# likojack/bnv_fusion

Measured on AMD Instinct MI355X. Metric: depth frames/sec fused+decoded, 640x480 @ 256^3 grid, higher is better.
Workload: dtype f32 operands split into f16 hi+lo, 3 products on v_mfma_f32_16x16x32_f16, f32 accumulate

## Files before the change

### bnv_fusion_amd/csrc/encode_mlp.hip

```cpp
#include "encode.hpp"

namespace bnv {

__device__ __forceinline__ f32x16 relu16(f32x16 v) {
#pragma unroll
  for (int r = 0; r < 16; ++r) v[r] = relu_bits(v[r]);
  return v;
}

__device__ __forceinline__ f32x16 bias_init(const float* __restrict__ b, int mb, int h) {
  f32x16 v;
#pragma unroll
  for (int q = 0; q < 4; ++q) {
    const f32x4 t = *(const f32x4*)&b[mb * 32 + 8 * q + 4 * h];
#pragma unroll
    for (int i = 0; i < 4; ++i) v[4 * q + i] = t[i];
  }
  return v;
}

__device__ __forceinline__ void layer128(const float* __restrict__ wp, const float* __restrict__ bias,
                                         const f32x16 (&in)[4], f32x16 (&out)[4], int lane, int h) {
#pragma unroll
  for (int mb = 0; mb < 4; ++mb) out[mb] = bias_init(bias, mb, h);
#pragma unroll
  for (int nb = 0; nb < 4; ++nb) {
#pragma unroll
    for (int rq = 0; rq < 4; ++rq) {
      f32x4 a[4];
#pragma unroll
      for (int mb = 0; mb < 4; ++mb)
        a[mb] = *(const f32x4*)&wp[(((mb * 4 + nb) * 4 + rq) * 64 + lane) * 4];
#pragma unroll
      for (int i = 0; i < 4; ++i) {
#pragma unroll
        for (int mb = 0; mb < 4; ++mb)
          out[mb] = __builtin_amdgcn_mfma_f32_32x32x2f32(a[mb][i], in[nb][4 * rq + i], out[mb], 0, 0, 0);
      }
    }
  }
}

__global__ __launch_bounds__(512, 2) void k_pointnet_scatter(
    const float* __restrict__ pts, int n_points, bnv_grid_t g, const float* __restrict__ wpack,
    const uint32_t* __restrict__ bitmap, const uint32_t* __restrict__ word_prefix,
    int32_t* __restrict__ counts, long long* __restrict__ acc, const int32_t* __restrict__ pair_list,
    const int32_t* __restrict__ n_pairs) {
  extern __shared__ __attribute__((aligned(16))) float lds[];
  stage_to_lds<512>(wpack, lds, PN_TOTAL * 4);
  __syncthreads();

  const int lane = threadIdx.x & 63;
  const int wave = __builtin_amdgcn_readfirstlane(threadIdx.x >> 6);
  const int j = lane & 31, h = lane >> 5;
  const PairTiles T = pair_tiles(n_points, pair_list, n_pairs);
  const int n_tiles = T.n_tiles;

  for (int t = blockIdx.x * 8 + wave; t < n_tiles; t += gridDim.x * 8) {
    int i = 0, k = 0;
    const bool have = tile_pair(T, t, j, &i, &k);
    float in0 = 0.f, in1 = 0.f, in2 = 0.f;
    int slot = -1;
    bool valid = false;
    if (have) {
      const float* p = pts + (size_t)i * 6;
      const float x = p[0], y = p[1], z = p[2];
      valid = in_bounds(x, y, z, g);
      if (valid) {
        const float xn = voxel_coord(x, g.bound_min[0], g.voxel_size);
        const float yn = voxel_coord(y, g.bound_min[1], g.voxel_size);
        const float zn = voxel_coord(z, g.bound_min[2], g.voxel_size);
        int gx, gy, gz;
        const uint32_t id = corner_voxel(k, xn, yn, zn, g, gx, gy, gz);
        if (voxel_owner(gx, gy, gz, g) == g.shard_rank) slot = slot_rank(bitmap[id >> 5], word_prefix[id >> 5], id);
        const float rx = relative_coord(xn, gx, g.voxel_size);
        const float ry = relative_coord(yn, gy, g.voxel_size);
        const float rz = relative_coord(zn, gz, g.voxel_size);
        in0 = h ? ry : rx;
        in1 = h ? p[3] : rz;
        in2 = h ? p[5] : p[4];
      }
    }
    if (__ballot(slot >= 0) == 0ULL) continue;

    f32x16 ha[4], hb[4];
#pragma unroll
    for (int mb = 0; mb < 4; ++mb) ha[mb] = bias_init(lds + PN_B1, mb, h);
    {
      const float bin[3] = {in0, in1, in2};
#pragma unroll
      for (int s = 0; s < 3; ++s) {
#pragma unroll
        for (int mb = 0; mb < 4; ++mb)
          ha[mb] = __builtin_amdgcn_mfma_f32_32x32x2f32(lds[PN_W1 + (s * 4 + mb) * 64 + lane], bin[s],
                                                        ha[mb], 0, 0, 0);
      }
    }
#pragma unroll
    for (int mb = 0; mb < 4; ++mb) ha[mb] = relu16(ha[mb]);
    layer128(lds + PN_W2, lds + PN_B2, ha, hb, lane, h);
#pragma unroll
    for (int mb = 0; mb < 4; ++mb) hb[mb] = relu16(hb[mb]);
    layer128(lds + PN_W3, lds + PN_B3, hb, ha, lane, h);
#pragma unroll
    for (int mb = 0; mb < 4; ++mb) ha[mb] = relu16(ha[mb]);
    f32x16 o;
#pragma unroll
    for (int r = 0; r < 16; ++r) o[r] = 0.f;
    {
      const f32x4 b4 = *(const f32x4*)&lds[PN_B4 + 4 * h];
#pragma unroll
      for (int r = 0; r < 4; ++r) o[r] = b4[r];
    }
#pragma unroll
    for (int nb = 0; nb < 4; ++nb) {
#pragma unroll
      for (int rq = 0; rq < 4; ++rq) {
        f32x4 a = {0.f, 0.f, 0.f, 0.f};
        if (j < 8) a = *(const f32x4*)&lds[PN_W4 + ((((nb * 4 + rq) * 2 + h) * 8) + j) * 4];
#pragma unroll
        for (int i = 0; i < 4; ++i)
          o = __builtin_amdgcn_mfma_f32_32x32x2f32(a[i], ha[nb][4 * rq + i], o, 0, 0, 0);
      }
    }
    scatter_tile(o, slot, j, h, counts, acc);
  }
}

typedef __attribute__((address_space(3))) const half8 lds_half8_t;
typedef __attribute__((address_space(3))) const f32x4 lds_f32x4_t;
constexpr int kLdsWin = 61440;

#ifdef BNV_PHASE_PROF
__device__ unsigned long long g_enc_phase[8 * 16];
#define BNV_EPH(i)                                                                          \
  do {                                                                                      \
    if ((threadIdx.x & 63) == 0) {                                                          \
      unsigned long long* _p = (unsigned long long*)((char*)lds + PX_LDS_BYTES) + (threadIdx.x >> 6) * 16; \
      const unsigned long long _t = clock64();                                              \
      _p[i] += _t - _p[15];                                                                 \
      _p[15] = _t;                                                                          \
    }                                                                                       \
  } while (0)
constexpr int kEncProfLds = 8 * 16 * 8;
#else
#define BNV_EPH(i)
constexpr int kEncProfLds = 0;
#endif

struct EncLdsX {
  uint32_t w[3];
  uint32_t b;
};
__device__ __forceinline__ half8 ldsx_wfrag(const EncLdsX& L, int byte_off) {
  const int b = byte_off / kLdsWin;
  return *(lds_half8_t*)((b == 0 ? L.w[0] : (b == 1 ? L.w[1] : L.w[2])) + (uint32_t)(byte_off - b * kLdsWin));
}
__device__ __forceinline__ f32x4 ldsx_bias(const EncLdsX& L, int layer, int rb) {
  return *(lds_f32x4_t*)(L.b + (uint32_t)((layer * 128 + rb * 16) * 4));
}

template <int NPROD>
__device__ __forceinline__ void layer128_x(const EncLdsX& L, int w_off, int layer, const half8 (&inh)[4][2],
                                           const half8 (&inl)[4][2], f32x4 (&out)[8][2]) {
#pragma unroll
  for (int rb = 0; rb < 8; ++rb) out[rb][0] = out[rb][1] = ldsx_bias(L, layer, rb);
  half8 ah[2], al[2];
#define BNV_LOAD_WX(q)                                                        \
  {                                                                           \
    const int wb = (w_off + (q) * 2 * 64 * 8) * 2;                            \
    ah[(q) & 1] = ldsx_wfrag(L, wb);                                          \
    if (NPROD == 3) al[(q) & 1] = ldsx_wfrag(L, wb + 1024);                   \
  }
  BNV_LOAD_WX(0);
#pragma unroll
  for (int q = 0; q < 32; ++q) {
    if (q + 1 < 32) BNV_LOAD_WX(q + 1);
    __builtin_amdgcn_sched_barrier(0);
    const int s = q >> 3, rb = q & 7;
    if constexpr (NPROD == 3) {
      out[rb][0] = __builtin_amdgcn_mfma_f32_16x16x32_f16(al[q & 1], inh[s][0], out[rb][0], 0, 0, 0);
      out[rb][1] = __builtin_amdgcn_mfma_f32_16x16x32_f16(al[q & 1], inh[s][1], out[rb][1], 0, 0, 0);
      out[rb][0] = __builtin_amdgcn_mfma_f32_16x16x32_f16(ah[q & 1], inl[s][0], out[rb][0], 0, 0, 0);
      out[rb][1] = __builtin_amdgcn_mfma_f32_16x16x32_f16(ah[q & 1], inl[s][1], out[rb][1], 0, 0, 0);
    }
    out[rb][0] = __builtin_amdgcn_mfma_f32_16x16x32_f16(ah[q & 1], inh[s][0], out[rb][0], 0, 0, 0);
    out[rb][1] = __builtin_amdgcn_mfma_f32_16x16x32_f16(ah[q & 1], inh[s][1], out[rb][1], 0, 0, 0);
    __builtin_amdgcn_sched_barrier(0);
  }
#undef BNV_LOAD_WX
}

template <int NPROD>
__device__ __forceinline__ void split_x(const f32x4 (&acc)[8][2], half8 (&oh)[4][2], half8 (&ol)[4][2]) {
#pragma unroll
  for (int s = 0; s < 4; ++s)
#pragma unroll
    for (int cb = 0; cb < 2; ++cb) {
      float x[8];
#pragma unroll
      for (int e = 0; e < 8; ++e) x[e] = relu_bits(acc[2 * s + (e >> 2)][cb][e & 3]);
      if (NPROD == 3) {
        split8_f16(x, oh[s][cb], ol[s][cb]);
      } else {
#pragma unroll
        for (int e = 0; e < 8; ++e) oh[s][cb][e] = (_Float16)x[e];
      }
    }
}

__device__ __forceinline__ void scatter_tile_x(const f32x4& o, int slot, int n, int g, int32_t* __restrict__ counts,
                                               long long* __restrict__ acc) {
  uint32_t lo[4], hi[4];
#pragma unroll
  for (int q = 0; q < 4; ++q) fixed_hi_lo(o[q], hi[q], lo[q]);
  asm volatile(BNV_SCAN_ROWS : BNV_SCAN_REGS(lo, hi) : : "vcc");
  {
    const int tsrc = ((g & 1) * 16 + 15) * 4;
#pragma unroll
    for (int q = 0; q < 4; ++q) {
      const uint32_t tl = (uint32_t)__builtin_amdgcn_ds_bpermute(tsrc, (int)lo[q]);
      const uint32_t th = (uint32_t)__builtin_amdgcn_ds_bpermute(tsrc, (int)hi[q]);
      if (g >= 2) {
        const unsigned long long v = (((unsigned long long)hi[q] << 32) | lo[q]) + (((unsigned long long)th << 32) | tl);
        lo[q] = (uint32_t)v;
        hi[q] = (uint32_t)(v >> 32);
      }
    }
  }
  const int p = (g >> 1) * 16 + n;
  const int slot15 = __builtin_amdgcn_readlane(slot, 15);
  const int prev_row = __builtin_amdgcn_update_dpp(0, slot, 0x111 , 0xf, 0xf, false);
  const int prev = n == 0 ? slot15 : prev_row;
  const unsigned long long heads64 = __ballot(p == 0 || prev != slot);
  const uint32_t heads = ((uint32_t)heads64 & 0xffffu) | (((uint32_t)(heads64 >> 32) & 0xffffu) << 16);
  const int s = 31 - __clz((int)(heads & (0xffffffffu >> (31 - p))));
  const bool is_end = p == 31 || ((heads >> (p + 1)) & 1u);
  const int sp = s > 0 ? s - 1 : 0;
  const int src = (((sp >> 4) * 2 + (g & 1)) * 16 + (sp & 15)) * 4;
  uint32_t plo[4], phi[4];
#pragma unroll
  for (int q = 0; q < 4; ++q) {
    plo[q] = (uint32_t)__builtin_amdgcn_ds_bpermute(src, (int)lo[q]);
    phi[q] = (uint32_t)__builtin_amdgcn_ds_bpermute(src, (int)hi[q]);
  }
#ifdef BNV_PROBE_NO_SCATTER
  if ((blockIdx.x & 63) != 0) return;
#endif
  if (slot >= 0 && is_end) {
    unsigned long long* dst = (unsigned long long*)acc + ((uint32_t)slot * 8u + 4u * (uint32_t)(g & 1));
#pragma unroll
    for (int q = 0; q < 4; ++q) {
      unsigned long long v = ((unsigned long long)hi[q] << 32) | lo[q];
      if (s > 0) v -= ((unsigned long long)phi[q] << 32) | plo[q];
      atomicAdd(dst + q, v);
    }
    if ((g & 1) == 0) atomicAdd(&counts[slot], p - s + 1);
  }
}

template <int NPROD>
__global__ __launch_bounds__(512, 2) __attribute__((amdgpu_num_vgpr(120))) void k_pointnet_scatter_x(
    const float* __restrict__ pts, int n_points, bnv_grid_t g, const float* __restrict__ wpack,
    const uint32_t* __restrict__ bitmap, const uint32_t* __restrict__ word_prefix,
    int32_t* __restrict__ counts, long long* __restrict__ acc, int32_t* __restrict__ error,
    const int32_t* __restrict__ pair_list, const int32_t* __restrict__ n_pairs) {
  extern __shared__ __attribute__((aligned(16))) float lds[];
  const float n_cert = wpack[PN_CERT];
  float* lb = lds + PX_TOTAL / 2;
  for (int i = threadIdx.x; i < 128 * 3 + 8; i += 512) lb[i] = wpack[PN_B1 + i];
  stage_to_lds<512>(wpack + PX_OFF, lds, PX_TOTAL * 2);
  int* tile_ctr = (int*)((char*)lds + PX_TOTAL * 2 + (128 * 3 + 8) * 4);
  if (threadIdx.x == 0) *tile_ctr = 0;
  __syncthreads();

  const int lane = threadIdx.x & 63;
  const int n = lane & 15, gk = lane >> 4;
  const int pair = (gk >> 1) * 16 + n;
  const PairTiles T = pair_tiles(n_points, pair_list, n_pairs);
  const int n_tiles = T.n_tiles;
  const int nyz = g.n_xyz[1] * g.n_xyz[2];
  EncLdsX L;
  {
    const uint32_t lds0 = (uint32_t)(uintptr_t)(__attribute__((address_space(3))) float*)lds;
    L.w[0] = lds0 + lane * 16;
    L.w[1] = L.w[0] + kLdsWin;
    L.w[2] = L.w[0] + 2 * kLdsWin;
    L.b = lds0 + PX_TOTAL * 2 + gk * 16;
    asm volatile("" : "+v"(L.w[0]), "+v"(L.w[1]), "+v"(L.w[2]), "+v"(L.b));
  }

  const int tstep = gridDim.x * 8;
  auto grab = [&]() -> int {
    int c = 0;
    if (lane == 0) c = atomicAdd(tile_ctr, 1);
    c = __builtin_amdgcn_readfirstlane(c);
    return blockIdx.x * 8 + (c & 7) + (c >> 3) * tstep;
  };
  float raw[6];
  int raw_k = 0;
  bool raw_ok = false;
  float nin[6];
  uint32_t n_id = 0, n_word = 0, n_pref = 0;
  bool n_own = false;
  auto stage1 = [&](int t) {
    raw_ok = false;
    if (t < n_tiles) {
      int i = 0;
      if (tile_pair(T, t, pair, &i, &raw_k)) {
        const float* p = pts + (size_t)i * 6;
#pragma unroll
        for (int c = 0; c < 6; ++c) raw[c] = p[c];
        raw_ok = true;
      }
    }
  };
  auto stage2 = [&](int t) {
    n_own = false;
#pragma unroll
    for (int c = 0; c < 6; ++c) nin[c] = 0.f;
    if (raw_ok && in_bounds(raw[0], raw[1], raw[2], g)) {
      const int k = raw_k;
      const float xn = voxel_coord(raw[0], g.bound_min[0], g.voxel_size);
      const float yn = voxel_coord(raw[1], g.bound_min[1], g.voxel_size);
      const float zn = voxel_coord(raw[2], g.bound_min[2], g.voxel_size);
      int gx, gy, gz;
      corner_xyz(k, xn, yn, zn, gx, gy, gz);
      if (voxel_owner(gx, gy, gz, g) == g.shard_rank) {
        n_own = true;
        n_id = voxel_id(gx, gy, gz, nyz, g.n_xyz[2]);
        n_word = bitmap[n_id >> 5];
        n_pref = word_prefix[n_id >> 5];
      }
      if ((gk & 1) == 0) {
        nin[0] = relative_coord(xn, gx, g.voxel_size);
        nin[1] = relative_coord(yn, gy, g.voxel_size);
        nin[2] = relative_coord(zn, gz, g.voxel_size);
        nin[3] = raw[3];
        nin[4] = raw[4];
        nin[5] = raw[5];
      }
      if (!(fmaxf(fmaxf(fabsf(raw[3]), fabsf(raw[4])), fabsf(raw[5])) <= n_cert)) *error = 3;
    }
  };
  int t = grab();
  stage1(t);
  stage2(t);
  int t_next = grab(), t_next2 = 0;
  stage1(t_next);
#ifdef BNV_PHASE_PROF
  if ((threadIdx.x & 63) < 16)
    ((unsigned long long*)((char*)lds + PX_LDS_BYTES))[(threadIdx.x >> 6) * 16 + (threadIdx.x & 63)] = 0;
  if ((threadIdx.x & 63) == 0) ((unsigned long long*)((char*)lds + PX_LDS_BYTES))[(threadIdx.x >> 6) * 16 + 15] = clock64();
#endif

  for (; t < n_tiles; t = t_next, t_next = t_next2) {
    float in[6];
#pragma unroll
    for (int c = 0; c < 6; ++c) in[c] = nin[c];
    const int slot = n_own ? slot_rank(n_word, n_pref, n_id) : -1;
    stage2(t_next);
    t_next2 = grab();
    stage1(t_next2);
    __builtin_amdgcn_sched_barrier(0);
    BNV_EPH(0);
    if (__ballot(slot >= 0) == 0ULL) continue;

    f32x4 ha[8][2], hb[8][2];
    {
      half8 bh[2], bl[2];
#pragma unroll
      for (int cb = 0; cb < 2; ++cb) {
        float x[8];
#pragma unroll
        for (int e = 0; e < 8; ++e) x[e] = 0.f;
#pragma unroll
        for (int e = 0; e < 6; ++e) {
          const float other = __shfl(in[e], (lane + 32) & 63, 64);
          x[e] = gk == 0 ? (cb == 0 ? in[e] : other) : 0.f;
        }
        if (NPROD == 3) {
          split8_f16(x, bh[cb], bl[cb]);
        } else {
#pragma unroll
          for (int e = 0; e < 8; ++e) bh[cb][e] = (_Float16)x[e];
        }
      }
#pragma unroll
      for (int rb = 0; rb < 8; ++rb) {
        const half8 ahi = ldsx_wfrag(L, (PX_W1 + rb * 2 * 64 * 8) * 2), alo = ldsx_wfrag(L, (PX_W1 + rb * 2 * 64 * 8) * 2 + 1024);
        const f32x4 b = ldsx_bias(L, 0, rb);
#pragma unroll
        for (int cb = 0; cb < 2; ++cb) {
          f32x4 c = b;
          if constexpr (NPROD == 3) {
            c = __builtin_amdgcn_mfma_f32_16x16x32_f16(alo, bh[cb], c, 0, 0, 0);
            c = __builtin_amdgcn_mfma_f32_16x16x32_f16(ahi, bl[cb], c, 0, 0, 0);
          }
          ha[rb][cb] = __builtin_amdgcn_mfma_f32_16x16x32_f16(ahi, bh[cb], c, 0, 0, 0);
        }
      }
    }
    BNV_EPH(1);
    half8 sh[4][2], sl[4][2];
    split_x<NPROD>(ha, sh, sl);
    BNV_EPH(2);
    layer128_x<NPROD>(L, PX_W2, 1, sh, sl, hb);
    BNV_EPH(3);
    split_x<NPROD>(hb, sh, sl);
    BNV_EPH(4);
    layer128_x<NPROD>(L, PX_W3, 2, sh, sl, ha);
    BNV_EPH(5);
    split_x<NPROD>(ha, sh, sl);
    BNV_EPH(6);
    f32x4 o[2];
    o[0] = o[1] = *(lds_f32x4_t*)(L.b + 384 * 4);
    {
      half8 w4h[4], w4l[4];
      __builtin_amdgcn_sched_barrier(0);
#pragma unroll
      for (int s = 0; s < 4; ++s) {
        w4h[s] = ldsx_wfrag(L, (PX_W4 + s * 2 * 64 * 8) * 2);
        if (NPROD == 3) w4l[s] = ldsx_wfrag(L, (PX_W4 + s * 2 * 64 * 8) * 2 + 1024);
      }
#pragma unroll
      for (int s = 0; s < 4; ++s) {
#pragma unroll
        for (int cb = 0; cb < 2; ++cb) {
          if constexpr (NPROD == 3) {
            o[cb] = __builtin_amdgcn_mfma_f32_16x16x32_f16(w4l[s], sh[s][cb], o[cb], 0, 0, 0);
            o[cb] = __builtin_amdgcn_mfma_f32_16x16x32_f16(w4h[s], sl[s][cb], o[cb], 0, 0, 0);
          }
          o[cb] = __builtin_amdgcn_mfma_f32_16x16x32_f16(w4h[s], sh[s][cb], o[cb], 0, 0, 0);
        }
      }
    }
    f32x4 mine;
#pragma unroll
    for (int i = 0; i < 4; ++i) {
      const float other = __shfl(o[1][i], (lane + 32) & 63, 64);
      mine[i] = gk < 2 ? o[0][i] : other;
    }
    BNV_EPH(7);
    scatter_tile_x(mine, slot, n, gk, counts, acc);
    BNV_EPH(8);
  }
#ifdef BNV_PHASE_PROF
  if ((threadIdx.x & 63) < 15)
    atomicAdd(&g_enc_phase[(threadIdx.x >> 6) * 16 + (threadIdx.x & 63)],
              ((unsigned long long*)((char*)lds + PX_LDS_BYTES))[(threadIdx.x >> 6) * 16 + (threadIdx.x & 63)]);
#endif
}

int encode_init() {
  const hipFuncAttribute lds = hipFuncAttributeMaxDynamicSharedMemorySize;
  BNV_HIP_CHECK(hipFuncSetAttribute((const void*)k_pointnet_scatter, lds, PN_TOTAL * 4));
  BNV_HIP_CHECK(hipFuncSetAttribute((const void*)k_pointnet_scatter_x<3>, lds, PX_LDS_BYTES + kEncProfLds));
  BNV_HIP_CHECK(hipFuncSetAttribute((const void*)k_pointnet_scatter_x<1>, lds, PX_LDS_BYTES + kEncProfLds));
  return BNV_OK;
}

void launch_encoder_mlp(int mlp, int grid, const float* pts, int n, const bnv_grid_t& g, const float* pack,
                        const EncodeWs& ws, const int32_t* plist, hipStream_t stream) {
  if (mlp == 1 || mlp == 3)
    hipLaunchKernelGGL(mlp == 1 ? k_pointnet_scatter_x<3> : k_pointnet_scatter_x<1>, dim3(grid), dim3(512),
                       PX_LDS_BYTES + kEncProfLds, stream, pts, n, g, pack, ws.bitmap, ws.word_prefix, ws.counts,
                       ws.acc, &ws.ctl->error, plist, &ws.ctl->n_pairs);
  else
    hipLaunchKernelGGL(k_pointnet_scatter, dim3(grid), dim3(512), PN_TOTAL * 4, stream, pts, n, g, pack, ws.bitmap,
                       ws.word_prefix, ws.counts, ws.acc, plist, &ws.ctl->n_pairs);
}

}

#ifdef BNV_PHASE_PROF
extern "C" int bnv_dev_enc_phase_read(unsigned long long* out128) {
  BNV_HIP_CHECK(hipDeviceSynchronize());
  BNV_HIP_CHECK(hipMemcpyFromSymbol(out128, HIP_SYMBOL(bnv::g_enc_phase), 128 * sizeof(unsigned long long)));
  unsigned long long z[128] = {};
  BNV_HIP_CHECK(hipMemcpyToSymbol(HIP_SYMBOL(bnv::g_enc_phase), z, sizeof(z)));
  return BNV_OK;
}
#endif
```

Baseline: 567.5.

## Interleave next-tile prefetch and coordinate stages into MFMA layer loops

```diff
diff --git a/bnv_fusion_amd/csrc/encode_mlp.hip b/bnv_fusion_amd/csrc/encode_mlp.hip
--- a/bnv_fusion_amd/csrc/encode_mlp.hip
+++ b/bnv_fusion_amd/csrc/encode_mlp.hip
@@ -160,9 +160,10 @@
   return *(lds_f32x4_t*)(L.b + (uint32_t)((layer * 128 + rb * 16) * 4));
 }
 
-template <int NPROD>
+constexpr int kFillPerMfma = 2;
+template <int NPROD, typename F>
 __device__ __forceinline__ void layer128_x(const EncLdsX& L, int w_off, int layer, const half8 (&inh)[4][2],
-                                           const half8 (&inl)[4][2], f32x4 (&out)[8][2]) {
+                                           const half8 (&inl)[4][2], f32x4 (&out)[8][2], F&& fill) {
 #pragma unroll
   for (int rb = 0; rb < 8; ++rb) out[rb][0] = out[rb][1] = ldsx_bias(L, layer, rb);
   half8 ah[2], al[2];
@@ -177,6 +178,7 @@
   for (int q = 0; q < 32; ++q) {
     if (q + 1 < 32) BNV_LOAD_WX(q + 1);
     __builtin_amdgcn_sched_barrier(0);
+    fill(q);
     const int s = q >> 3, rb = q & 7;
     if constexpr (NPROD == 3) {
       out[rb][0] = __builtin_amdgcn_mfma_f32_16x16x32_f16(al[q & 1], inh[s][0], out[rb][0], 0, 0, 0);
@@ -186,6 +188,11 @@
     }
     out[rb][0] = __builtin_amdgcn_mfma_f32_16x16x32_f16(ah[q & 1], inh[s][0], out[rb][0], 0, 0, 0);
     out[rb][1] = __builtin_amdgcn_mfma_f32_16x16x32_f16(ah[q & 1], inh[s][1], out[rb][1], 0, 0, 0);
+#pragma unroll
+    for (int m = 0; m < 2 * NPROD; ++m) {
+      __builtin_amdgcn_sched_group_barrier(0x008, 1, 0);
+      __builtin_amdgcn_sched_group_barrier(0x012, kFillPerMfma, 0);
+    }
     __builtin_amdgcn_sched_barrier(0);
   }
 #undef BNV_LOAD_WX
@@ -290,81 +297,124 @@
     asm volatile("" : "+v"(L.w[0]), "+v"(L.w[1]), "+v"(L.w[2]), "+v"(L.b));
   }
 
+  if (n_tiles == 0) return;
   const int tstep = gridDim.x * 8;
-  auto grab = [&]() -> int {
-    int c = 0;
-    if (lane == 0) c = atomicAdd(tile_ctr, 1);
-    c = __builtin_amdgcn_readfirstlane(c);
-    return blockIdx.x * 8 + (c & 7) + (c >> 3) * tstep;
-  };
+  const bool listed = T.list != nullptr;
+  const int32_t* lbase = listed ? T.list : n_pairs;
+  const int n_pblocks = T.n_pblocks > 0 ? T.n_pblocks : 1;
+  int grab_c = 0;
+  int lent = 0;
+  bool lent_ok = false;
   float raw[6];
   int raw_k = 0;
   bool raw_ok = false;
   float nin[6];
   uint32_t n_id = 0, n_word = 0, n_pref = 0;
   bool n_own = false;
-  auto stage1 = [&](int t) {
-    raw_ok = false;
-    if (t < n_tiles) {
-      int i = 0;
-      if (tile_pair(T, t, pair, &i, &raw_k)) {
-        const float* p = pts + (size_t)i * 6;
-#pragma unroll
-        for (int c = 0; c < 6; ++c) raw[c] = p[c];
-        raw_ok = true;
-      }
-    }
-  };
-  auto stage2 = [&](int t) {
-    n_own = false;
-#pragma unroll
-    for (int c = 0; c < 6; ++c) nin[c] = 0.f;
-    if (raw_ok && in_bounds(raw[0], raw[1], raw[2], g)) {
-      const int k = raw_k;
-      const float xn = voxel_coord(raw[0], g.bound_min[0], g.voxel_size);
-      const float yn = voxel_coord(raw[1], g.bound_min[1], g.voxel_size);
-      const float zn = voxel_coord(raw[2], g.bound_min[2], g.voxel_size);
-      int gx, gy, gz;
-      corner_xyz(k, xn, yn, zn, gx, gy, gz);
-      if (voxel_owner(gx, gy, gz, g) == g.shard_rank) {
-        n_own = true;
+  int slot_next = -1, bad = 0;
+  int t = 0, t_next = 0, t_next2 = 0;
+  float sx = 0.f, sy = 0.f, sz = 0.f, xn = 0.f, yn = 0.f, zn = 0.f;
+  int gx = 0, gy = 0, gz = 0;
+  bool s_ok = false, take = false;
+  auto grab_issue = [&]() {
+    grab_c = 0;
+    if (lane == 0) grab_c = (int)atomicInc((unsigned*)tile_ctr, 0xffffffffu);
+  };
+  auto grab_finish = [&]() -> int {
+    const int c = __builtin_amdgcn_readfirstlane(grab_c);
+    return blockIdx.x * 8 + (c & 7) + (c >> 3) * tstep;
+  };
+  auto list_issue = [&](int tile) {
+    const int e = tile * 32 + pair;
+    lent_ok = listed & ((unsigned)tile < (unsigned)n_tiles) & (e < T.n_pairs);
+    lent = lbase[lent_ok ? e : 0];
+  };
+  auto point_issue = [&](int tile) {
+    const int ku = tile / n_pblocks;
+    const int iu = (tile - ku * n_pblocks) * 32 + pair;
+    const int i = listed ? lent >> 3 : iu;
+    raw_k = listed ? lent & 7 : ku;
+    raw_ok = listed ? lent_ok : (((unsigned)tile < (unsigned)n_tiles) & (iu < T.n_points));
+    const float* p = pts + (size_t)(raw_ok ? i : 0) * 6;
+#pragma unroll
+    for (int c = 0; c < 6; ++c) raw[c] = p[c];
+  };
+  auto pin = [](auto& x) __attribute__((always_inline)) { asm volatile("" : "+v"(x)); };
+  auto stage = [&](int c) __attribute__((always_inline)) {
+    switch (c) {
+      case 0: grab_issue(); break;
+      case 2:
+        s_ok = raw_ok & in_bounds(raw[0], raw[1], raw[2], g);
+        sx = s_ok ? raw[0] : g.bound_min[0];
+        sy = s_ok ? raw[1] : g.bound_min[1];
+        sz = s_ok ? raw[2] : g.bound_min[2];
+        take = s_ok & ((gk & 1) == 0);
+        break;
+      case 3: xn = voxel_coord(sx, g.bound_min[0], g.voxel_size); break;
+      case 4: yn = voxel_coord(sy, g.bound_min[1], g.voxel_size); break;
+      case 5: zn = voxel_coord(sz, g.bound_min[2], g.voxel_size); break;
+      case 6: corner_xyz(raw_k, xn, yn, zn, gx, gy, gz); break;
+      case 7: {
+        n_own = s_ok & (voxel_owner(gx, gy, gz, g) == g.shard_rank);
         n_id = voxel_id(gx, gy, gz, nyz, g.n_xyz[2]);
-        n_word = bitmap[n_id >> 5];
-        n_pref = word_prefix[n_id >> 5];
-      }
-      if ((gk & 1) == 0) {
-        nin[0] = relative_coord(xn, gx, g.voxel_size);
-        nin[1] = relative_coord(yn, gy, g.voxel_size);
-        nin[2] = relative_coord(zn, gz, g.voxel_size);
-        nin[3] = raw[3];
-        nin[4] = raw[4];
-        nin[5] = raw[5];
-      }
-      if (!(fmaxf(fmaxf(fabsf(raw[3]), fabsf(raw[4])), fabsf(raw[5])) <= n_cert)) *error = 3;
-    }
-  };
-  int t = grab();
-  stage1(t);
-  stage2(t);
-  int t_next = grab(), t_next2 = 0;
-  stage1(t_next);
+        const uint32_t w = n_own ? n_id >> 5 : 0u;
+        n_word = bitmap[w];
+        n_pref = word_prefix[w];
+        break;
+      }
+      case 8:
+        t_next2 = grab_finish();
+        list_issue(t_next2);
+        break;
+      case 9: { const float r = relative_coord(xn, gx, g.voxel_size); nin[0] = take ? r : 0.f; pin(nin[0]); break; }
+      case 10: { const float r = relative_coord(yn, gy, g.voxel_size); nin[1] = take ? r : 0.f; pin(nin[1]); break; }
+      case 11: { const float r = relative_coord(zn, gz, g.voxel_size); nin[2] = take ? r : 0.f; pin(nin[2]); break; }
+      case 12:
+#pragma unroll
+        for (int e = 3; e < 6; ++e) { nin[e] = take ? raw[e] : 0.f; pin(nin[e]); }
+        bad |= (int)(s_ok & !(fmaxf(fmaxf(fabsf(raw[3]), fabsf(raw[4])), fabsf(raw[5])) <= n_cert));
+        pin(bad);
+        break;
+      case 34: point_issue(t_next2); break;
+      case 60: slot_next = n_own ? slot_rank(n_word, n_pref, n_id) : -1; pin(slot_next); pin(n_word); pin(n_pref); break;
+      default: break;
+    }
+  };
+  auto stage_all = [&]() {
+    constexpr int used[] = {0, 2, 3, 4, 5, 6, 7, 8, 9, 10, 11, 12, 34, 60};
+#pragma unroll
+    for (int c : used) stage(c);
+  };
+  auto settle = [&]() {
+#pragma unroll
+    for (int c = 0; c < 6; ++c) pin(raw[c]);
+    pin(n_word), pin(n_pref), pin(lent);
+  };
+  grab_issue();
+  t_next2 = grab_finish();
+  list_issue(t_next2);
+  point_issue(t_next2);
+  t_next = t_next2;
+  stage_all();
+  settle();
+  t = t_next, t_next = t_next2;
+  int slot = slot_next;
 #ifdef BNV_PHASE_PROF
   if ((threadIdx.x & 63) < 16)
     ((unsigned long long*)((char*)lds + PX_LDS_BYTES))[(threadIdx.x >> 6) * 16 + (threadIdx.x & 63)] = 0;
   if ((threadIdx.x & 63) == 0) ((unsigned long long*)((char*)lds + PX_LDS_BYTES))[(threadIdx.x >> 6) * 16 + 15] = clock64();
 #endif
 
-  for (; t < n_tiles; t = t_next, t_next = t_next2) {
+  for (; t < n_tiles; t = t_next, t_next = t_next2, slot = slot_next) {
     float in[6];
 #pragma unroll
     for (int c = 0; c < 6; ++c) in[c] = nin[c];
-    const int slot = n_own ? slot_rank(n_word, n_pref, n_id) : -1;
-    stage2(t_next);
-    t_next2 = grab();
-    stage1(t_next2);
-    __builtin_amdgcn_sched_barrier(0);
     BNV_EPH(0);
-    if (__ballot(slot >= 0) == 0ULL) continue;
+    if (__ballot(slot >= 0) == 0ULL) {
+      stage_all();
+      settle();
+      continue;
+    }
 
     f32x4 ha[8][2], hb[8][2];
     {
@@ -405,11 +455,11 @@
     half8 sh[4][2], sl[4][2];
     split_x<NPROD>(ha, sh, sl);
     BNV_EPH(2);
-    layer128_x<NPROD>(L, PX_W2, 1, sh, sl, hb);
+    layer128_x<NPROD>(L, PX_W2, 1, sh, sl, hb, [&](int q) __attribute__((always_inline)) { stage(q); });
     BNV_EPH(3);
     split_x<NPROD>(hb, sh, sl);
     BNV_EPH(4);
-    layer128_x<NPROD>(L, PX_W3, 2, sh, sl, ha);
+    layer128_x<NPROD>(L, PX_W3, 2, sh, sl, ha, [&](int q) __attribute__((always_inline)) { stage(32 + q); });
     BNV_EPH(5);
     split_x<NPROD>(ha, sh, sl);
     BNV_EPH(6);
@@ -441,10 +491,12 @@
       const float other = __shfl(o[1][i], (lane + 32) & 63, 64);
       mine[i] = gk < 2 ? o[0][i] : other;
     }
+    settle();
     BNV_EPH(7);
     scatter_tile_x(mine, slot, n, gk, counts, acc);
     BNV_EPH(8);
   }
+  if (bad) *error = 3;
 #ifdef BNV_PHASE_PROF
   if ((threadIdx.x & 63) < 15)
     atomicAdd(&g_enc_phase[(threadIdx.x >> 6) * 16 + (threadIdx.x & 63)],
```

Measured after the change: 564.0. No clear change (-0.6%).
